# zdebruine/singlet

Measured on AMD Instinct MI355X. Metric: ALS iterations/sec (1M cells x 30k genes, 5% nnz, k=50), higher is better.
Workload: dtype f64

## Files before the change

### include/singlet_hip.h

```cpp
#ifndef SINGLET_HIP_H
#define SINGLET_HIP_H

#include <stddef.h>
#include <stdint.h>

#ifdef __cplusplus
extern "C" {
#endif

#define SGL_API __attribute__((visibility("default")))

#define SGL_OK 0
#define SGL_EINVAL (-1)
#define SGL_ENODEV (-2)
#define SGL_EHIP (-3)
#define SGL_ENOMEM (-4)
#define SGL_EINTR (-5)
#define SGL_ESTATE (-6)
#define SGL_ECOMM (-7)

SGL_API const char* sgl_last_error(void);
SGL_API int sgl_abi_version(void);
SGL_API int sgl_device_count(void);

// ... 282 lines not shown
SGL_API int sgl_comm_info(sgl_ctx* ctx, int32_t* nranks, int32_t* is_rccl, char* path_out, int path_len);
SGL_API int sgl_split_cells_by_nnz(const int32_t* p, int32_t ncol, int n, int64_t* lo);

SGL_API int sgl_op_rand(sgl_ctx* ctx, uint64_t state, const uint64_t* i, const uint64_t* j, int64_t n, uint64_t* out);
SGL_API int sgl_op_mask(sgl_ctx* ctx, uint64_t state, uint64_t inv_density, int64_t cell0, int32_t ncells, int32_t ngenes,
                uint8_t* out);
SGL_API int sgl_op_gram(sgl_ctx* ctx, const double* F, int32_t k, int64_t cols, double* G);
SGL_API int sgl_op_mask_gram(sgl_ctx* ctx, const double* F, const double* G, int32_t k, int32_t nrow, int64_t ncols, uint64_t seed,
                uint64_t inv_density, int mask_t, int64_t col_offset, int64_t row_offset, int use_lists, double* out);
SGL_API int sgl_op_rhs(sgl_ctx* ctx, int which, const double* F, int32_t k, double* B);
SGL_API int sgl_op_nnls(sgl_ctx* ctx, const double* G, const double* B, double* X, int32_t k, int64_t ncols,
                double L1, double L2, int32_t* sweeps_out);
SGL_API int sgl_op_transpose(sgl_ctx* ctx, int64_t max_batch_entries);
SGL_API int sgl_op_scale(sgl_ctx* ctx, double* F, int32_t k, int64_t cols, double* d);
SGL_API int sgl_op_cor(sgl_ctx* ctx, const double* x, const double* y, int64_t n, double* out);
SGL_API int sgl_op_graph_conv(sgl_ctx* ctx, const double* X, int32_t k, double* Y);
SGL_API int sgl_op_mse_test(sgl_ctx* ctx, uint64_t seed, uint64_t inv_density, double* out);
SGL_API int sgl_op_rhs_masked(sgl_ctx* ctx, int which, const double* F, int32_t k, uint64_t seed, uint64_t inv_density, double* B);
SGL_API int sgl_op_gene_mean(sgl_ctx* ctx, double* mean, int64_t* count);
SGL_API int sgl_op_gene_var(sgl_ctx* ctx, const double* mu, double* var);
SGL_API int sgl_op_gene_var_std(sgl_ctx* ctx, const double* mu, const double* sd, double vmax, double* out);
SGL_API int sgl_op_loess_direct(sgl_ctx* ctx, const double* x, const double* y, int64_t n, int64_t q, double* fitted);
SGL_API int sgl_op_marker_sums(sgl_ctx* ctx, const int32_t* labels, int32_t n_groups, int transform, int64_t* pos, int64_t* nz, double* sum);
SGL_API int sgl_op_marker_ranks(sgl_ctx* ctx, const int32_t* labels, int32_t n_groups, int64_t max_batch_entries, int64_t* rank2,
                                uint64_t* tie);
SGL_API int sgl_op_gsea_es(sgl_ctx* ctx, const double* w, int32_t m, int32_t k, const int64_t* set_ptr, const int32_t* set_genes,
                           int32_t n_sets, double* es_pos, double* es_neg, double* es_std);
SGL_API int sgl_op_gsea_null(sgl_ctx* ctx, const double* w, int32_t m, int32_t k, const int32_t* sizes, int32_t n_sizes,
                             int score_type, uint64_t seed, int32_t r0, int32_t r1, int32_t batch, double* null_out,
                             int32_t* sample);
// ... 28 lines not shown
```

### singlet_amd/_lib.py

```python
import ctypes as C
import os

_HERE = os.path.dirname(os.path.abspath(__file__))
LIB_PATH = os.environ.get("SGL_LIB_PATH", os.path.join(_HERE, "libsinglet_hip.so"))

SGL_PH_NAMES = ("gram", "rhs_h", "nnls_h", "rhs_w", "nnls_w", "scale", "comm", "mask", "mse")
SGL_PH_COUNT = len(SGL_PH_NAMES)

f64p = C.POINTER(C.c_double)
i32p = C.POINTER(C.c_int32)
i64p = C.POINTER(C.c_int64)
u64p = C.POINTER(C.c_uint64)
u8p = C.POINTER(C.c_uint8)

LOG_FN = C.CFUNCTYPE(None, C.c_void_p, C.c_int, C.c_double, C.c_double)
POLL_FN = C.CFUNCTYPE(C.c_int, C.c_void_p)
ALLREDUCE_FN = C.CFUNCTYPE(C.c_int, C.c_void_p, C.c_void_p, C.c_int64)


class Callbacks(C.Structure):
    _fields_ = [("user", C.c_void_p), ("log", LOG_FN), ("poll", POLL_FN)]


class SingletHipError(RuntimeError):
# ... 137 lines not shown
    "sgl_comm_available": (C.c_int, [C.c_char_p, C.c_int]),
    "sgl_comm_info": (C.c_int, [C.c_void_p, i32p, i32p, C.c_char_p, C.c_int]),
    "sgl_split_cells_by_nnz": (C.c_int, [i32p, C.c_int32, C.c_int, i64p]),
    "sgl_get_factors": (C.c_int, [C.c_void_p, f64p, f64p, f64p]),
    "sgl_set_factors": (C.c_int, [C.c_void_p, f64p, f64p, f64p]),
    "sgl_op_rand": (C.c_int, [C.c_void_p, C.c_uint64, u64p, u64p, C.c_int64, u64p]),
    "sgl_op_mask": (C.c_int, [C.c_void_p, C.c_uint64, C.c_uint64, C.c_int64, C.c_int32, C.c_int32, u8p]),
    "sgl_op_gram": (C.c_int, [C.c_void_p, f64p, C.c_int32, C.c_int64, f64p]),
    "sgl_op_rhs": (C.c_int, [C.c_void_p, C.c_int, f64p, C.c_int32, f64p]),
    "sgl_op_nnls": (C.c_int, [C.c_void_p, f64p, f64p, f64p, C.c_int32, C.c_int64, C.c_double, C.c_double, i32p]),
    "sgl_op_mask_gram": (C.c_int, [C.c_void_p, f64p, f64p, C.c_int32, C.c_int32, C.c_int64, C.c_uint64, C.c_uint64, C.c_int, C.c_int64,
                                   C.c_int64, C.c_int, f64p]),
    "sgl_op_transpose": (C.c_int, [C.c_void_p, C.c_int64]),
    "sgl_op_scale": (C.c_int, [C.c_void_p, f64p, C.c_int32, C.c_int64, f64p]),
    "sgl_op_cor": (C.c_int, [C.c_void_p, f64p, f64p, C.c_int64, f64p]),
    "sgl_op_graph_conv": (C.c_int, [C.c_void_p, f64p, C.c_int32, f64p]),
    "sgl_op_mse_test": (C.c_int, [C.c_void_p, C.c_uint64, C.c_uint64, f64p]),
    "sgl_op_rhs_masked": (C.c_int, [C.c_void_p, C.c_int, f64p, C.c_int32, C.c_uint64, C.c_uint64, f64p]),
    "sgl_op_gene_mean": (C.c_int, [C.c_void_p, f64p, i64p]),
    "sgl_op_gene_var": (C.c_int, [C.c_void_p, f64p, f64p]),
    "sgl_op_gene_var_std": (C.c_int, [C.c_void_p, f64p, f64p, C.c_double, f64p]),
    "sgl_op_loess_direct": (C.c_int, [C.c_void_p, f64p, f64p, C.c_int64, C.c_int64, f64p]),
    "sgl_op_nnls_percol": (C.c_int, [C.c_void_p, f64p, f64p, f64p, i64p, C.c_int32, C.c_int64, C.c_double, C.c_double, i32p]),
    "sgl_op_mse_test_cells": (C.c_int, [C.c_void_p, C.c_uint64, C.c_uint64, C.c_int, f64p]),
    "sgl_timing_enable": (C.c_int, [C.c_void_p, C.c_int]),
    "sgl_timing_get": (C.c_int, [C.c_void_p, f64p, i64p, C.c_int]),
    "sgl_sweeps_get": (C.c_int, [C.c_void_p, i64p, C.c_int]),
    "sgl_layout_get": (C.c_int, [C.c_void_p, i64p]),
    "sgl_layout_builds": (C.c_int, [C.c_void_p, i64p]),
    "sgl_mask_pairs": (C.c_int, [C.c_void_p, i64p]),
# ... 38 lines not shown
```

### singlet_amd/context.py

```python
import ctypes as C

import numpy as np

from . import _lib
from ._lib import check, f64p, i32p, i64p, ptr, u64p, u8p
from ._marshal import (MARKER_TRANSFORMS, ArdOutputs, NmfOutputs, colmajor, csc_ptrs, gsea_inputs, gsea_score_type, knn_call, label_list,
                       markers_call)
from .sparse import as_dgCMatrix

SYNTH_SEED = 0x5EED
LEVELS16 = np.log1p(1.0 + np.arange(16, dtype=np.float64))


def skew_weights16(sigma):
    z = np.array([-1.8627318674, -1.3180108973, -1.0099901692, -0.7764217611, -0.5791321623, -0.4022500653, -0.2372021093, -0.0784124127])
    z = np.concatenate([z, -z[::-1]])
    w = np.exp(float(sigma) * z)
    return w / w.mean()


def _f(a):
    return np.ascontiguousarray(a, dtype=np.float64)


# ... 506 lines not shown
        check(self._L.sgl_op_mask_gram(self._h, ptr(F, f64p), Gp, k, nrow, ncols, int(seed), int(inv_density), int(mask_t),
                                       int(col_offset), int(row_offset), 1 if use_lists else 0, ptr(out, f64p)))
        return out

    def op_transpose(self, max_batch_entries=0):
        check(self._L.sgl_op_transpose(self._h, int(max_batch_entries)))
        self.k = 0

    def op_scale(self, F):
        F = np.array(F, dtype=np.float64, order="C")
        cols, k = F.shape
        d = np.empty(k)
        check(self._L.sgl_op_scale(self._h, ptr(F, f64p), k, cols, ptr(d, f64p)))
        return F, d

    def op_cor(self, x, y):
        x, y = _f(x), _f(y)
        out = C.c_double()
        check(self._L.sgl_op_cor(self._h, ptr(x, f64p), ptr(y, f64p), x.size, C.byref(out)))
        return out.value

    def op_graph_conv(self, X, out=None):
        X = _f(X)
        n, k = X.shape
        _, nc, _ = self.dims()
        if n != nc:
            raise ValueError("X must have %d rows (the cells of the resident matrix)" % nc)
        Y = np.empty((n, k)) if out is None else out
        if Y.shape != (n, k) or Y.dtype != np.float64 or not Y.flags.c_contiguous:
            raise ValueError("out must be a C-contiguous float64 array of X's shape")
# ... 202 lines not shown
```

### singlet_amd/csrc/kernels_dense.hip

```cpp
#include "sgl_internal.h"

typedef double d4 __attribute__((ext_vector_type(4)));

template <int NT>
__global__ __launch_bounds__(256) void gram_mfma_kernel(const double* __restrict__ F, int k, int64_t cols,
                                                        int64_t cols_per_block, double* __restrict__ part) {
    constexpr int NTILES = NT * (NT + 1) / 2;
    const int lane = threadIdx.x & 63, wave = threadIdx.x >> 6;
    const int r16 = lane & 15, kk = lane >> 4;
    const int64_t c_begin = (int64_t)blockIdx.x * cols_per_block;
    int64_t c_end = c_begin + cols_per_block;
    if (c_end > cols) c_end = cols;

    d4 acc[NTILES];
#pragma unroll
    for (int t = 0; t < NTILES; ++t) acc[t] = d4{0, 0, 0, 0};

    for (int64_t c = c_begin + 4 * wave; c < c_end; c += 16) {
        const int64_t cc = c + kk;
        double f[NT];
#pragma unroll
        for (int b = 0; b < NT; ++b) {
            const int row = b * 16 + r16;
            f[b] = (cc < c_end && row < k) ? F[cc * k + row] : 0.0;
        }
        int t = 0;
#pragma unroll
        for (int bi = 0; bi < NT; ++bi)
#pragma unroll
            for (int bj = 0; bj <= bi; ++bj) {
                acc[t] = __builtin_amdgcn_mfma_f64_16x16x4f64(f[bi], f[bj], acc[t], 0, 0, 0);
                ++t;
            }
    }

    __shared__ double sm[4][64 * 4];
    double* out = part + (size_t)blockIdx.x * k * k;
    int t = 0;
#pragma unroll
    for (int bi = 0; bi < NT; ++bi)
#pragma unroll
        for (int bj = 0; bj <= bi; ++bj) {
            __syncthreads();
#pragma unroll
            for (int r = 0; r < 4; ++r) sm[wave][lane * 4 + r] = acc[t][r];
            __syncthreads();
            if (wave == 0) {
#pragma unroll
// ... 170 lines not shown
        partial_sum_small_kernel<<<dim3(1), dim3(1024), 0, c->stream>>>(c->ws, nblocks, n, nseg, add_all, out);
        HIPCHK(hipGetLastError());
        return SGL_OK;
    }
    if (add_all != 0.0) { sgl_set_error("partial sum: add_all only in the short form"); return SGL_EINVAL; }
    double* tmp = c->ws + (size_t)nblocks * n;
    partial_sum_stage1_kernel<<<dim3((n + 255) / 256, nseg), dim3(256), 0, c->stream>>>(c->ws, nblocks, n, tmp);
    HIPCHK(hipGetLastError());
    partial_sum_stage2_kernel<<<dim3((n + 255) / 256), dim3(256), 0, c->stream>>>(tmp, nseg, n, diag_k, diag_add, out);
    HIPCHK(hipGetLastError());
    return SGL_OK;
}

int k_gram_big_partials(hipStream_t s, const double* F, int k, int64_t cols, int64_t cols_per_block, int nblocks, double* part);

int k_gram(sgl_ctx* c, const double* F, int k, int64_t cols, double* G, double diag_add) {
    if (k <= 0 || k > SGL_MAX_K) { sgl_set_error("k_gram: k=%d out of range", k); return SGL_EINVAL; }
    int nblocks = (int)((cols + 255) / 256);
    if (nblocks > 1024) nblocks = 1024;
    const bool big_mfma = k > 128 && k <= 256 && !getenv("SGL_GRAM_BIG_VALU");
    if (k > 128 && nblocks > (big_mfma ? 512 : 128)) nblocks = big_mfma ? 512 : 128;
    if (nblocks < 1) nblocks = 1;
    int64_t cpb = (cols + nblocks - 1) / nblocks;
    cpb = (cpb + 15) / 16 * 16;
    nblocks = (int)((cols + cpb - 1) / cpb);
    if (nblocks < 1) nblocks = 1;
    SGLCHK(sgl_ws_reserve(c, sizeof(double) * sgl_partial_ws(nblocks, k * k)));
    hipStream_t s = c->stream;
    const int NT = (k + 15) / 16;
    if (NT == 1) gram_mfma_kernel<1><<<dim3(nblocks), dim3(256), 0, s>>>(F, k, cols, cpb, c->ws);
    else if (NT == 2) gram_mfma_kernel<2><<<dim3(nblocks), dim3(256), 0, s>>>(F, k, cols, cpb, c->ws);
    else if (NT == 3) gram_mfma_kernel<3><<<dim3(nblocks), dim3(256), 0, s>>>(F, k, cols, cpb, c->ws);
    else if (NT == 4) gram_mfma_kernel<4><<<dim3(nblocks), dim3(256), 0, s>>>(F, k, cols, cpb, c->ws);
    else if (NT == 5) gram_mfma_split_kernel<5><<<dim3(nblocks), dim3(256), 0, s>>>(F, k, cols, cpb, c->ws);
    else if (NT == 6) gram_mfma_split_kernel<6><<<dim3(nblocks), dim3(256), 0, s>>>(F, k, cols, cpb, c->ws);
    else if (NT == 7) gram_mfma_split_kernel<7><<<dim3(nblocks), dim3(256), 0, s>>>(F, k, cols, cpb, c->ws);
    else if (NT == 8) gram_mfma_split_kernel<8><<<dim3(nblocks), dim3(256), 0, s>>>(F, k, cols, cpb, c->ws);
    else if (big_mfma) SGLCHK(k_gram_big_partials(s, F, k, cols, cpb, nblocks, c->ws));
    else {
        const size_t lds = sizeof(double) * 16 * (size_t)k;
        if (lds > 48 * 1024) HIPCHK(hipFuncSetAttribute(reinterpret_cast<const void*>(&gram_valu_kernel), hipFuncAttributeMaxDynamicSharedMemorySize, 144 * 1024));
        for (int pair0 = 0; pair0 < k * k; pair0 += 256 * GV_MAXP)
            gram_valu_kernel<<<dim3(nblocks), dim3(256), lds, s>>>(F, k, cols, cpb, c->ws, pair0);
    }
    HIPCHK(hipGetLastError());
    return sgl_partial_sum(c, nblocks, k * k, k, diag_add, G);
}

// ... 72 lines not shown

int k_scale_apply(hipStream_t s, double* F, int k, int64_t cols, double* d, int add_eps) {
    if (add_eps) {
        add_eps_kernel<<<dim3((k + 63) / 64), dim3(64), 0, s>>>(d, k);
        HIPCHK(hipGetLastError());
    }
    const int64_t n = (int64_t)k * cols;
    if (n <= 0) return SGL_OK;
    int64_t blocks = (n + 255) / 256;
    if (blocks > 4096) blocks = 4096;
    scale_kernel<<<dim3((unsigned)blocks), dim3(256), 0, s>>>(F, k, n, d);
    HIPCHK(hipGetLastError());
    return SGL_OK;
}

__global__ __launch_bounds__(256) void cor_partial_kernel(const double* __restrict__ x, const double* __restrict__ y,
                                                          int64_t n, double* __restrict__ part) {
    double s[5] = {0, 0, 0, 0, 0};
    for (int64_t t = (int64_t)blockIdx.x * blockDim.x + threadIdx.x; t < n; t += (int64_t)gridDim.x * blockDim.x) {
        const double a = x[t], b = y[t];
        s[0] += a;
        s[1] += b;
        s[2] = fma(a, b, s[2]);
        s[3] = fma(a, a, s[3]);
        s[4] = fma(b, b, s[4]);
    }
    __shared__ double sm[5][256];
    for (int q = 0; q < 5; ++q) sm[q][threadIdx.x] = s[q];
    __syncthreads();
    for (int w = 128; w > 0; w >>= 1) {
// ... 122 lines not shown
```

### singlet_amd/csrc/sgl_internal.h

```cpp
#pragma once
#include <hip/hip_runtime.h>
#include <stdint.h>
#include <stdio.h>
#include <stdarg.h>
#include <atomic>
#include <functional>
#include <vector>
#include <algorithm>

#include "../../include/singlet_hip.h"

#define SGL_WAVE 64
#define SGL_MAX_K 1024
#define SGL_LANE_NNLS_MAX_K 128

void sgl_set_error(const char* fmt, ...);

hipError_t sgl_pool_malloc_raw(void** p, size_t bytes);
template <typename T_>
inline hipError_t sgl_pool_malloc(T_** p, size_t bytes) { return sgl_pool_malloc_raw(reinterpret_cast<void**>(p), bytes); }
hipError_t sgl_pool_free(void* p);
hipError_t sgl_pool_mem_info(size_t* free_b, size_t* total_b);
void sgl_pool_release(void);
size_t sgl_pool_cached_bytes(void);
// ... 150 lines not shown
    hipStream_t stream = nullptr;

    DevCSC A, At;
    DevTiled TA, TAt;
    bool use_tiled = false;
    int64_t cell_offset = 0, ncells_total = 0;
    int64_t* col_nnz_A = nullptr;
    int64_t* col_nnz_At = nullptr;
    int64_t* col_nnz_At_global = nullptr;
    bool gene_nnz_global = false;

    int k = 0;
    double *W = nullptr, *Wprev = nullptr, *H = nullptr, *d = nullptr;
    double* B = nullptr;
    double* red = nullptr;
    double* G = nullptr;
    double* Gpad = nullptr;
    NnlsScratch nnls_scr;
    bool solve_empty = false;
    double* Adense = nullptr;
    bool dense_gemm = false;
    void* rocblas = nullptr;
    double* link_h = nullptr;
    double* link_w = nullptr;
    int link_h_rows = 0, link_w_rows = 0;
    DevGroupLink glink_h, glink_w;
    DevGraph graph;
    bool dense_input = false;
    DevMaskList ML[2];
    int64_t ml_builds[2] = {0, 0};
// ... 118 lines not shown
                 const double* skew_dev = nullptr);
int k_synth_winit(hipStream_t s, uint64_t S, int k, int32_t ngenes, double* W);
int k_exclusive_scan(sgl_ctx* c, const int64_t* in, int64_t* out, int64_t n);
int k_scan_total(hipStream_t s, const int64_t* in, int64_t* out, int64_t n);
int k_col_counts(hipStream_t s, const int64_t* p, int64_t ncol, int64_t* counts);
int k_validate_csc(hipStream_t s, const int32_t* idx, const int64_t* p, int64_t ncol, int32_t nrow, int* flag_dev);
int k_all_finite(hipStream_t s, const double* x, int64_t n, int* flag_dev);
int k_widen_p(hipStream_t s, const int32_t* p32, int64_t n1, int64_t* p64);
int k_build_segments(hipStream_t s, const DevCSC& M);

int k_gram(sgl_ctx* c, const double* F, int k, int64_t cols, double* G, double diag_add);
int k_gram_add_diag(hipStream_t s, double* G, int k, double v);
int k_rowsum(sgl_ctx* c, const double* F, int k, int64_t cols, double* d_out, int add_eps = 0);
bool k_rowsum_can_add_eps(int k, int64_t cols);
int k_scale_apply(hipStream_t s, double* F, int k, int64_t cols, double* d, int add_eps);
int k_cor(sgl_ctx* c, const double* x, const double* y, int64_t n, double* out_dev);
int k_pad_gram(hipStream_t s, const double* G, int k, int KP, int GS, double* Gpad);
int k_gram_rescale(hipStream_t s, double* G, int k, const double* d, double diag_add);
int k_i64_to_f64(hipStream_t s, const int64_t* in, double* out, int64_t n);
int k_f64_to_i64(hipStream_t s, const double* in, int64_t* out, int64_t n);
int k_transpose_dense(hipStream_t s, const double* in, int rows, int cols, double* out);

int k_acc(hipStream_t s, const DevCSC& M, const double* F, int k, double* B,
          uint64_t mask_seed, uint64_t inv_density, int mask_mode, int64_t mask_col_offset, int64_t mask_row_offset);

void sgl_tiled_free(DevTiled& S);
int sgl_tiled_build(sgl_ctx* c, const DevCSC& M, int k, DevTiled& S);
int k_acc_tiled(hipStream_t s, const DevTiled& S, const double* F, int ldf, double* B, int ldb, int kf, const double* xvals = nullptr);
int k_acc_tiled_all(hipStream_t s, const DevTiled& S, const double* F, double* B, int k, const double* xvals = nullptr);
int sgl_tiled_mask_values(sgl_ctx* c, const DevCSC& M, DevTiled& S, uint64_t seed, uint64_t inv_density, int mask_t,
// ... 167 lines not shown
```

### singlet_amd/csrc/singlet_hip.hip

```cpp
#include "sgl_internal.h"
#include "ingest_host.h"

#include <math.h>
#include <string.h>
#include <algorithm>
#include <string>
#include <chrono>
#include <mutex>
#include <vector>
#include <stdlib.h>

static thread_local char g_err[1024] = "";

void sgl_set_error(const char* fmt, ...) {
    va_list ap;
    va_start(ap, fmt);
    vsnprintf(g_err, sizeof(g_err), fmt, ap);
    va_end(ap);
}

extern "C" const char* sgl_last_error(void) { return g_err; }
extern "C" int sgl_abi_version(void) { return 2; }

struct CallTimes {
// ... 143 lines not shown
    dev_free(c->Wd);
    dev_free(c->Sbuf);
    dev_free(c->Stri);
    nnls_scratch_free(c->nnls_scr);
    links_clear(c);
    free_graph(c);
    dev_free(c->A.seg);
    dev_free(c->At.seg);
    if (!keep_streams) {
        sgl_tiled_free(c->TA);
        sgl_tiled_free(c->TAt);
        sgl_mask_lists_free_all(c);
    }
    c->use_tiled = false;
    c->k = 0;
}

static void free_matrix(sgl_ctx* c) {
    sgl_dense_release(c);
    free_csc(c->A);
    free_csc(c->At);
    dev_free(c->col_nnz_A);
    dev_free(c->col_nnz_At);
    dev_free(c->col_nnz_At_global);
    c->gene_nnz_global = false;
    c->dense_input = false;
}

static int drop_matrix(sgl_ctx* c, int rc) {
    (void)hipStreamSynchronize(c->stream);
// ... 755 lines not shown
    if (rc == SGL_OK) rc = sgl_download_csc(c, 0, x_out, nullptr, nullptr);
    sgl_destroy(c);
    return rc;
}

static int64_t team_gene_block(const sgl_ctx* c) {
    const int64_t m = c->A.nrow;
    const int n = sgl_team_size(c);
    return n > 1 ? (m + n - 1) / n : m;
}

static int fit_init_impl(sgl_ctx* c, int32_t k, const double* w_init, uint64_t synth_seed) {
    const int64_t m = c->A.nrow, n = c->A.ncol;
    const int64_t mpad = team_gene_block(c) * std::max(1, sgl_team_size(c));
    sgl_trace_setup(nullptr);
    SGLCHK(dev_alloc(&c->W, (size_t)k * mpad + 2));
    SGLCHK(dev_alloc(&c->Wprev, (size_t)k * m));
    SGLCHK(dev_alloc(&c->H, (size_t)k * n + 2));
    SGLCHK(dev_alloc(&c->d, (size_t)k));
    SGLCHK(dev_alloc(&c->B, (size_t)k * n + 2));
    SGLCHK(dev_alloc(&c->red, (size_t)k * mpad + (size_t)k * k + (size_t)k));
    SGLCHK(dev_alloc(&c->G, (size_t)k * k));
    SGLCHK(dev_alloc(&c->Gpad, (size_t)SGL_LANE_NNLS_MAX_K * (SGL_LANE_NNLS_MAX_K + 16) + 64));
    {
        const int64_t cap = std::max<int64_t>(c->A.ncol, c->A.nrow);
        if (k <= SGL_LANE_NNLS_MAX_K) SGLCHK(nnls_scratch_alloc(c->nnls_scr, cap, k));
        if (k <= 256 && c->A.ncol >= 65536) SGLCHK(nnls_pack_alloc(c->nnls_scr, c->A.ncol));
    }
    sgl_trace_setup("fit: factor buffers allocated");
    HIPCHK(hipMemsetAsync(c->W, 0, sizeof(double) * ((size_t)k * mpad + 2), c->stream));
// ... 93 lines not shown
    if (k > SGL_LANE_NNLS_MAX_K && k <= 256 && h_side && ncols == c->A.ncol && ncols >= 65536 && c->nnls_scr.prev_it != nullptr &&
        !getenv("SGL_NNLS_NO_QUARTER"))
        return k_nnls_quarter_packed(c->stream, G, B, X, col_nnz, k, ncols, L1, L2, counter, &c->nnls_scr);
    return k_nnls_percol(c->stream, G, 0, B, X, col_nnz, k, ncols, L1, L2, counter);
}

extern "C" int sgl_step_begin(sgl_ctx* c) {
    FIT_GUARD(c);
    Phase ph(c, SGL_PH_SCALE);
    HIPCHK(hipMemcpyAsync(c->Wprev, c->W, sizeof(double) * (size_t)c->k * c->A.nrow, hipMemcpyDeviceToDevice, c->stream));
    return SGL_OK;
}

int sgl_step_h_rhs(sgl_ctx* c, bool convolve) {
    const int k = c->k;
    { Phase ph(c, SGL_PH_GRAM); SGLCHK(k_gram(c, c->W, k, c->A.nrow, c->G, 1e-15)); }
    { Phase ph(c, SGL_PH_RHS_H);
      if (c->dense_gemm) SGLCHK(k_dense_rhs(c, 0, c->W, k, c->B));
      else if (c->use_tiled) SGLCHK(k_acc_tiled_all(c->stream, c->TA, c->W, c->B, k));
      else SGLCHK(k_acc(c->stream, c->A, c->W, k, c->B, 0, 1, 0, 0, 0));
      if (c->link_h) SGLCHK(k_link_mul(c->stream, c->B, c->link_h, k, c->link_h_rows, c->A.ncol));
      else if (c->glink_h.table) SGLCHK(k_link_mul_grouped(c->stream, c->B, c->glink_h.table, c->glink_h.group, k, c->glink_h.rows, c->glink_h.groups, c->A.ncol));
      if (c->graph.n && convolve) SGLCHK(k_graph_conv(c->stream, c->graph, c->B, c->graph.buf, k)); }
    return SGL_OK;
}

int sgl_step_h_solve(sgl_ctx* c, double L1, double L2, bool convolve) {
    const int k = c->k;
    if (c->graph.n && convolve) { Phase ph(c, SGL_PH_RHS_H); SGLCHK(k_graph_conv(c->stream, c->graph, c->B, c->graph.buf, k)); }
    { Phase ph(c, SGL_PH_NNLS_H);
      if (c->graph.n) SGLCHK(sgl_nnls_shared(c, c->G, c->graph.buf, c->H, nullptr, c->A.ncol, L1, L2, c->sweep_counters + 0, true));
      else SGLCHK(sgl_nnls_shared(c, c->G, c->B, c->H, c->solve_empty ? nullptr : c->col_nnz_A, c->A.ncol, L1, L2, c->sweep_counters + 0, true)); }
    return SGL_OK;
}

extern "C" int sgl_step_h(sgl_ctx* c, double L1, double L2) {
    FIT_GUARD(c);
    SGLCHK(sgl_step_h_rhs(c, true));
    return sgl_step_h_solve(c, L1, L2, false);
}

extern "C" int sgl_step_scale_h(sgl_ctx* c) {
    FIT_GUARD(c);
    if (c->team && sgl_team_size(c) > 1) { sgl_set_error("step API on a native team: use sgl_nmf_iterate / sgl_multi_iterate"); return SGL_ESTATE; }
    const int eps_in_sum = (!c->allreduce && k_rowsum_can_add_eps(c->k, c->A.ncol)) ? 1 : 0;
    { Phase ph(c, SGL_PH_SCALE); SGLCHK(k_rowsum(c, c->H, c->k, c->A.ncol, c->d, eps_in_sum)); }
    SGLCHK(do_allreduce(c, c->d, c->k));
    { Phase ph(c, SGL_PH_SCALE); SGLCHK(k_scale_apply(c->stream, c->H, c->k, c->A.ncol, c->d, eps_in_sum ? 0 : 1)); }
    return SGL_OK;
}

extern "C" int sgl_step_w(sgl_ctx* c, double L1, double L2) {
    FIT_GUARD(c);
    if (c->team && sgl_team_size(c) > 1) { sgl_set_error("step API on a native team: use sgl_nmf_iterate / sgl_multi_iterate"); return SGL_ESTATE; }
    const int k = c->k;
    const int64_t m = c->A.nrow;
    double* Bw = c->red;
    double* Gh = c->red + (size_t)k * m;
    const int64_t* gene_nnz = nullptr;
    SGLCHK(gene_counts(c, &gene_nnz));
    { Phase ph(c, SGL_PH_RHS_W);
      const double* F = c->H;
      if (c->graph.n) { SGLCHK(k_graph_conv(c->stream, c->graph, c->H, c->B, k)); F = c->B; }
      if (c->dense_gemm) SGLCHK(k_dense_rhs(c, 1, F, k, Bw));
      else if (c->use_tiled && c->TAt.roff) SGLCHK(k_acc_tiled_all(c->stream, c->TAt, F, Bw, k));
      else SGLCHK(k_acc(c->stream, c->At, F, k, Bw, 0, 1, 0, 0, 0)); }
    { Phase ph(c, SGL_PH_GRAM); SGLCHK(k_gram(c, c->H, k, c->A.ncol, Gh, 0.0)); }
    SGLCHK(do_allreduce(c, c->red, (int64_t)k * m + (int64_t)k * k));
    { Phase ph(c, SGL_PH_GRAM);
      HIPCHK(hipMemcpyAsync(c->G, Gh, sizeof(double) * k * k, hipMemcpyDeviceToDevice, c->stream));
      SGLCHK(k_gram_add_diag(c->stream, c->G, k, 1e-15)); }
    { Phase ph(c, SGL_PH_NNLS_W);
      if (c->link_w) SGLCHK(k_link_mul(c->stream, Bw, c->link_w, k, c->link_w_rows, m));
      else if (c->glink_w.table) SGLCHK(k_link_mul_grouped(c->stream, Bw, c->glink_w.table, c->glink_w.group, k, c->glink_w.rows, c->glink_w.groups, m));
      SGLCHK(sgl_nnls_shared(c, c->G, Bw, c->W, (c->solve_empty || c->graph.n) ? nullptr : gene_nnz, m, L1, L2, c->sweep_counters + 1)); }
    return SGL_OK;
}

int sgl_scale_w_enqueue(sgl_ctx* c) {
    const int k = c->k;
    const int64_t m = c->A.nrow;
    Phase ph(c, SGL_PH_SCALE);
// ... 27 lines not shown
    c->wave_sweeps_acc[0] += h[2];
    c->wave_sweeps_acc[1] += h[3];
    return SGL_OK;
}

static bool interrupted(const sgl_callbacks* cb) {
    if (!(cb && cb->poll && cb->poll(cb->user))) return false;
    sgl_set_error("interrupted");
    return true;
}

int sgl_iterate_shard(sgl_ctx* c, double L1_w, double L1_h, double L2_w, double L2_h, const ArdArgs* mask, const sgl_callbacks* cb,
                      double* tol) {
    SGLCHK(sgl_step_begin(c));
    SGLCHK(mask ? sgl_step_h_masked(c, L1_h, L2_h, mask->seed, mask->inv_density) : sgl_step_h(c, L1_h, L2_h));
    SGLCHK(sgl_step_scale_h(c));
    if (interrupted(cb)) return SGL_EINTR;
    SGLCHK(mask ? sgl_step_w_masked(c, L1_w, L2_w, mask->seed, mask->inv_density) : sgl_step_w(c, L1_w, L2_w));
    return sgl_step_scale_w(c, tol);
}

int sgl_als_loop(double tol, int32_t maxit, const std::function<int(double*)>& iterate, const ArdArgs* ard,
                 const std::function<int(double*)>& mse_test, sgl_ctx* const* ctxs, int nctx, double* tol_trace, int32_t* n_iter,
                 const sgl_callbacks* cb) {
    double tol_ = 1.0;
    int it = 0, nt = 0;
    auto push_trace = [&](int iter_now) -> int {
        double err = 0.0;
        SGLCHK(mse_test(&err));
        ard->test_mse[nt] = err;
        ard->iter[nt] = iter_now;
// ... 43 lines not shown
    HIPCHK(hipStreamSynchronize(c->stream));
    return SGL_OK;
}

extern "C" int sgl_get_factors(sgl_ctx* c, double* w, double* d, double* h) {
    FIT_GUARD(c);
    HIPCHK(hipStreamSynchronize(c->stream));
    if (w) HIPCHK(hipMemcpy(w, c->W, sizeof(double) * (size_t)c->k * c->A.nrow, hipMemcpyDeviceToHost));
    if (d) HIPCHK(hipMemcpy(d, c->d, sizeof(double) * (size_t)c->k, hipMemcpyDeviceToHost));
    if (h) HIPCHK(hipMemcpy(h, c->H, sizeof(double) * (size_t)c->k * c->A.ncol, hipMemcpyDeviceToHost));
    return SGL_OK;
}

extern "C" int sgl_set_factors(sgl_ctx* c, const double* w, const double* d, const double* h) {
    FIT_GUARD(c);
    HIPCHK(hipStreamSynchronize(c->stream));
    if (w) HIPCHK(hipMemcpy(c->W, w, sizeof(double) * (size_t)c->k * c->A.nrow, hipMemcpyHostToDevice));
    if (d) HIPCHK(hipMemcpy(c->d, d, sizeof(double) * (size_t)c->k, hipMemcpyHostToDevice));
    if (h) HIPCHK(hipMemcpy(c->H, h, sizeof(double) * (size_t)c->k * c->A.ncol, hipMemcpyHostToDevice));
    return SGL_OK;
}

int sgl_mask_workspace(sgl_ctx* c) {
    const int k = c->k;
    if (!c->Gcols) {
        const int64_t widest = std::max<int64_t>(c->A.ncol, c->At.ncol);
        size_t free_b = 0, total_b = 0;
        HIPCHK(sgl_pool_mem_info(&free_b, &total_b));
        const char* e = getenv("SGL_GCOLS_MB");
        const int64_t mb = (e && atoll(e) > 0) ? atoll(e) : std::min<int64_t>(16384, std::max<int64_t>(256, (int64_t)(free_b >> 23)));
// ... 12 lines not shown
    const DevCSC& M = orientation ? c->At : c->A;
    DevTiled& S = orientation ? c->TAt : c->TA;
    const int64_t col_off = mask_t ? 0 : c->cell_offset;
    const int64_t row_off = mask_t ? c->cell_offset : 0;
    if (c->use_tiled && S.roff && !getenv("SGL_MASKED_RHS_PLAIN")) {
        SGLCHK(sgl_tiled_mask_values(c, M, S, seed, inv_density, mask_t, col_off, row_off));
        return k_acc_tiled_all(c->stream, S, F, Bbuf, c->k, S.xm);
    }
    return k_acc(c->stream, M, F, c->k, Bbuf, seed, inv_density, mask_t ? 2 : 1, col_off, row_off);
}

int sgl_predict_mask_dev(sgl_ctx* c, const DevCSC& M, const int64_t* col_nnz, const double* F, double* X,
                            double* Bbuf, uint64_t seed, uint64_t inv_density, double L1, double L2, int mask_t,
                            int rhs_phase, int nnls_phase, unsigned long long* counter) {
    const int k = c->k;
    SGLCHK(sgl_mask_workspace(c));
    const int64_t col_off = mask_t ? 0 : c->cell_offset;
    const int64_t row_off = mask_t ? c->cell_offset : 0;
    { Phase ph(c, SGL_PH_GRAM); SGLCHK(k_gram(c, F, k, M.nrow, c->G, 1e-15)); }
    { Phase ph(c, rhs_phase);
      SGLCHK(sgl_masked_rhs(c, mask_t, F, Bbuf, seed, inv_density)); }
    const int64_t chunk = c->gcols_chunk;
    DevMaskList* L = nullptr;
    if (k <= 128 && !getenv("SGL_MASK_NO_LIST")) {
        Phase ph(c, SGL_PH_MASK);
        DevMaskList& Lm = c->ML[mask_t ? 1 : 0];
        SGLCHK(sgl_mask_list_select(c, mask_t ? 1 : 0, M.ncol, M.nrow, seed, inv_density, mask_t, col_off, row_off));
        if (Lm.mask_t == mask_t) L = &Lm;
    }
    for (int64_t c0 = 0; c0 < M.ncol; c0 += chunk) {
// ... 1055 lines not shown

extern "C" int sgl_op_scale(sgl_ctx* c, double* F, int32_t k, int64_t cols, double* d) {
    CTX_GUARD(c);
    if (!F || !d || k <= 0 || cols < 0) { sgl_set_error("sgl_op_scale: bad arguments"); return SGL_EINVAL; }
    DevBuf<double> dF, dd;
    SGLCHK(dF.alloc((size_t)k * cols));
    SGLCHK(dd.alloc((size_t)k));
    HIPCHK(hipMemcpyAsync(dF.p, F, sizeof(double) * (size_t)k * cols, hipMemcpyHostToDevice, c->stream));
    int rc = k_rowsum(c, dF.p, k, cols, dd.p);
    if (rc == SGL_OK) rc = k_scale_apply(c->stream, dF.p, k, cols, dd.p, 1);
    if (rc == SGL_OK && (hipMemcpyAsync(F, dF.p, sizeof(double) * (size_t)k * cols, hipMemcpyDeviceToHost, c->stream) != hipSuccess ||
                         hipMemcpyAsync(d, dd.p, sizeof(double) * (size_t)k, hipMemcpyDeviceToHost, c->stream) != hipSuccess)) rc = SGL_EHIP;
    return op_finish(c, rc, "sgl_op_scale");
}

extern "C" int sgl_op_cor(sgl_ctx* c, const double* x, const double* y, int64_t n, double* out) {
    CTX_GUARD(c);
    if (!x || !y || !out || n <= 0) { sgl_set_error("sgl_op_cor: bad arguments"); return SGL_EINVAL; }
    DevBuf<double> dx, dy;
    SGLCHK(dx.alloc((size_t)n));
    SGLCHK(dy.alloc((size_t)n));
    HIPCHK(hipMemcpyAsync(dx.p, x, sizeof(double) * (size_t)n, hipMemcpyHostToDevice, c->stream));
    HIPCHK(hipMemcpyAsync(dy.p, y, sizeof(double) * (size_t)n, hipMemcpyHostToDevice, c->stream));
    int rc = k_cor(c, dx.p, dy.p, n, c->scalars + 2);
    if (rc == SGL_OK && hipMemcpyAsync(out, c->scalars + 2, sizeof(double), hipMemcpyDeviceToHost, c->stream) != hipSuccess) rc = SGL_EHIP;
    return op_finish(c, rc, "sgl_op_cor");
}

extern "C" int sgl_op_graph_conv(sgl_ctx* c, const double* X, int32_t k, double* Y) {
    FIT_GUARD(c);
// ... 77 lines not shown
```

Before: 43.09.

## Fuse H scaling with H Gram computation and prefetch columns in gram kernel

Adds a SCALE variant of the MFMA gram kernel that divides each H column by d, writes it back and accumulates the Gram in the same pass. The W step then reuses the cached H Gram through a validity flag instead of recomputing it. This removes one full read/write pass over H (scale) plus a separate Gram read. The gram kernel also gains a register prefetch ring of depth SGL_GRAM_AHEAD, which hides load latency at the cost of extra registers. The cache flag must be invalidated on every path that mutates H, so missing an invalidation would reuse a stale Gram.

```diff
diff --git a/include/singlet_hip.h b/include/singlet_hip.h
--- a/include/singlet_hip.h
+++ b/include/singlet_hip.h
@@ -320,6 +320,7 @@
 SGL_API int sgl_op_transpose(sgl_ctx* ctx, int64_t max_batch_entries);
 SGL_API int sgl_op_scale(sgl_ctx* ctx, double* F, int32_t k, int64_t cols, double* d);
 SGL_API int sgl_op_cor(sgl_ctx* ctx, const double* x, const double* y, int64_t n, double* out);
+SGL_API int sgl_op_scale_gram(sgl_ctx* ctx, double* F, int32_t k, int64_t cols, double* d, double* G);
 SGL_API int sgl_op_graph_conv(sgl_ctx* ctx, const double* X, int32_t k, double* Y);
 SGL_API int sgl_op_mse_test(sgl_ctx* ctx, uint64_t seed, uint64_t inv_density, double* out);
 SGL_API int sgl_op_rhs_masked(sgl_ctx* ctx, int which, const double* F, int32_t k, uint64_t seed, uint64_t inv_density, double* B);
diff --git a/singlet_amd/_lib.py b/singlet_amd/_lib.py
--- a/singlet_amd/_lib.py
+++ b/singlet_amd/_lib.py
@@ -175,6 +175,7 @@
     "sgl_op_transpose": (C.c_int, [C.c_void_p, C.c_int64]),
     "sgl_op_scale": (C.c_int, [C.c_void_p, f64p, C.c_int32, C.c_int64, f64p]),
     "sgl_op_cor": (C.c_int, [C.c_void_p, f64p, f64p, C.c_int64, f64p]),
+    "sgl_op_scale_gram": (C.c_int, [C.c_void_p, f64p, C.c_int32, C.c_int64, f64p, f64p]),
     "sgl_op_graph_conv": (C.c_int, [C.c_void_p, f64p, C.c_int32, f64p]),
     "sgl_op_mse_test": (C.c_int, [C.c_void_p, C.c_uint64, C.c_uint64, f64p]),
     "sgl_op_rhs_masked": (C.c_int, [C.c_void_p, C.c_int, f64p, C.c_int32, C.c_uint64, C.c_uint64, f64p]),
diff --git a/singlet_amd/context.py b/singlet_amd/context.py
--- a/singlet_amd/context.py
+++ b/singlet_amd/context.py
@@ -544,6 +544,14 @@
         check(self._L.sgl_op_scale(self._h, ptr(F, f64p), k, cols, ptr(d, f64p)))
         return F, d
 
+    def op_scale_gram(self, F):
+        F = np.array(F, dtype=np.float64, order="C")
+        cols, k = F.shape
+        d = np.empty(k)
+        G = np.empty((k, k))
+        check(self._L.sgl_op_scale_gram(self._h, ptr(F, f64p), k, cols, ptr(d, f64p), ptr(G, f64p)))
+        return F, d, G
+
     def op_cor(self, x, y):
         x, y = _f(x), _f(y)
         out = C.c_double()
diff --git a/singlet_amd/csrc/kernels_dense.hip b/singlet_amd/csrc/kernels_dense.hip
--- a/singlet_amd/csrc/kernels_dense.hip
+++ b/singlet_amd/csrc/kernels_dense.hip
@@ -2,10 +2,18 @@
 
 typedef double d4 __attribute__((ext_vector_type(4)));
 
-template <int NT>
-__global__ __launch_bounds__(256) void gram_mfma_kernel(const double* __restrict__ F, int k, int64_t cols,
-                                                        int64_t cols_per_block, double* __restrict__ part) {
+#ifndef SGL_GRAM_AHEAD
+#define SGL_GRAM_AHEAD 2
+#endif
+template <bool SCALE> struct gram_operand { typedef const double* __restrict__ ptr; };
+template <> struct gram_operand<true> { typedef double* ptr; };
+
+template <int NT, bool SCALE>
+__global__ __launch_bounds__(256) void gram_mfma_kernel(typename gram_operand<SCALE>::ptr F, int k, int64_t cols,
+                                                        int64_t cols_per_block, const double* __restrict__ d,
+                                                        double* __restrict__ part) {
     constexpr int NTILES = NT * (NT + 1) / 2;
+    constexpr int AH = SGL_GRAM_AHEAD;
     const int lane = threadIdx.x & 63, wave = threadIdx.x >> 6;
     const int r16 = lane & 15, kk = lane >> 4;
     const int64_t c_begin = (int64_t)blockIdx.x * cols_per_block;
@@ -16,22 +24,56 @@
 #pragma unroll
     for (int t = 0; t < NTILES; ++t) acc[t] = d4{0, 0, 0, 0};
 
-    for (int64_t c = c_begin + 4 * wave; c < c_end; c += 16) {
-        const int64_t cc = c + kk;
-        double f[NT];
-#pragma unroll
-        for (int b = 0; b < NT; ++b) {
-            const int row = b * 16 + r16;
-            f[b] = (cc < c_end && row < k) ? F[cc * k + row] : 0.0;
-        }
-        int t = 0;
-#pragma unroll
-        for (int bi = 0; bi < NT; ++bi)
-#pragma unroll
-            for (int bj = 0; bj <= bi; ++bj) {
-                acc[t] = __builtin_amdgcn_mfma_f64_16x16x4f64(f[bi], f[bj], acc[t], 0, 0, 0);
-                ++t;
+    double dv[NT];
+#pragma unroll
+    for (int b = 0; b < NT; ++b) {
+        const int row = b * 16 + r16;
+        dv[b] = (SCALE && row < k) ? d[row] : 1.0;
+    }
+
+    double q[AH + 1][NT];
+    int64_t roff[NT];
+#pragma unroll
+    for (int b = 0; b < NT; ++b) roff[b] = (b * 16 + r16 < k) ? b * 16 + r16 : k - 1;
+    if (c_begin < c_end) {
+#pragma unroll
+        for (int a = 0; a < AH; ++a) {
+            const int64_t cc = c_begin + 4 * wave + 16 * a + kk;
+            const int64_t cl = (cc < c_end) ? cc : c_end - 1;
+#pragma unroll
+            for (int b = 0; b < NT; ++b) q[a][b] = F[cl * k + roff[b]];
+        }
+    }
+    for (int64_t c = c_begin + 4 * wave; c < c_end;) {
+#pragma unroll
+        for (int j = 0; j <= AH; ++j) {
+            if (c >= c_end) break;
+            const int64_t cc = c + kk, cn = cc + 16 * AH;
+            const int64_t cl = (cn < c_end) ? cn : c_end - 1;
+            double* nxt = q[(j + AH) % (AH + 1)];
+#pragma unroll
+            for (int b = 0; b < NT; ++b) nxt[b] = F[cl * k + roff[b]];
+            double f[NT];
+#pragma unroll
+            for (int b = 0; b < NT; ++b) {
+                const bool mine = cc < c_end && b * 16 + r16 < k;
+                f[b] = q[j][b];
+                if constexpr (SCALE) {
+                    f[b] = f[b] / dv[b];
+                    if (mine) F[cc * k + b * 16 + r16] = f[b];
+                }
+                f[b] = mine ? f[b] : 0.0;
             }
+            int t = 0;
+#pragma unroll
+            for (int bi = 0; bi < NT; ++bi)
+#pragma unroll
+                for (int bj = 0; bj <= bi; ++bj) {
+                    acc[t] = __builtin_amdgcn_mfma_f64_16x16x4f64(f[bi], f[bj], acc[t], 0, 0, 0);
+                    ++t;
+                }
+            c += 16;
+        }
     }
 
     __shared__ double sm[4][64 * 4];
@@ -232,24 +274,32 @@
 
 int k_gram_big_partials(hipStream_t s, const double* F, int k, int64_t cols, int64_t cols_per_block, int nblocks, double* part);
 
-int k_gram(sgl_ctx* c, const double* F, int k, int64_t cols, double* G, double diag_add) {
-    if (k <= 0 || k > SGL_MAX_K) { sgl_set_error("k_gram: k=%d out of range", k); return SGL_EINVAL; }
+static void gram_partition(int k, int64_t cols, bool big_mfma, int* nblocks_out, int64_t* cpb_out) {
     int nblocks = (int)((cols + 255) / 256);
     if (nblocks > 1024) nblocks = 1024;
-    const bool big_mfma = k > 128 && k <= 256 && !getenv("SGL_GRAM_BIG_VALU");
     if (k > 128 && nblocks > (big_mfma ? 512 : 128)) nblocks = big_mfma ? 512 : 128;
     if (nblocks < 1) nblocks = 1;
     int64_t cpb = (cols + nblocks - 1) / nblocks;
     cpb = (cpb + 15) / 16 * 16;
     nblocks = (int)((cols + cpb - 1) / cpb);
     if (nblocks < 1) nblocks = 1;
+    *nblocks_out = nblocks;
+    *cpb_out = cpb;
+}
+
+int k_gram(sgl_ctx* c, const double* F, int k, int64_t cols, double* G, double diag_add) {
+    if (k <= 0 || k > SGL_MAX_K) { sgl_set_error("k_gram: k=%d out of range", k); return SGL_EINVAL; }
+    const bool big_mfma = k > 128 && k <= 256 && !getenv("SGL_GRAM_BIG_VALU");
+    int nblocks;
+    int64_t cpb;
+    gram_partition(k, cols, big_mfma, &nblocks, &cpb);
     SGLCHK(sgl_ws_reserve(c, sizeof(double) * sgl_partial_ws(nblocks, k * k)));
     hipStream_t s = c->stream;
     const int NT = (k + 15) / 16;
-    if (NT == 1) gram_mfma_kernel<1><<<dim3(nblocks), dim3(256), 0, s>>>(F, k, cols, cpb, c->ws);
-    else if (NT == 2) gram_mfma_kernel<2><<<dim3(nblocks), dim3(256), 0, s>>>(F, k, cols, cpb, c->ws);
-    else if (NT == 3) gram_mfma_kernel<3><<<dim3(nblocks), dim3(256), 0, s>>>(F, k, cols, cpb, c->ws);
-    else if (NT == 4) gram_mfma_kernel<4><<<dim3(nblocks), dim3(256), 0, s>>>(F, k, cols, cpb, c->ws);
+    if (NT == 1) gram_mfma_kernel<1, false><<<dim3(nblocks), dim3(256), 0, s>>>(F, k, cols, cpb, nullptr, c->ws);
+    else if (NT == 2) gram_mfma_kernel<2, false><<<dim3(nblocks), dim3(256), 0, s>>>(F, k, cols, cpb, nullptr, c->ws);
+    else if (NT == 3) gram_mfma_kernel<3, false><<<dim3(nblocks), dim3(256), 0, s>>>(F, k, cols, cpb, nullptr, c->ws);
+    else if (NT == 4) gram_mfma_kernel<4, false><<<dim3(nblocks), dim3(256), 0, s>>>(F, k, cols, cpb, nullptr, c->ws);
     else if (NT == 5) gram_mfma_split_kernel<5><<<dim3(nblocks), dim3(256), 0, s>>>(F, k, cols, cpb, c->ws);
     else if (NT == 6) gram_mfma_split_kernel<6><<<dim3(nblocks), dim3(256), 0, s>>>(F, k, cols, cpb, c->ws);
     else if (NT == 7) gram_mfma_split_kernel<7><<<dim3(nblocks), dim3(256), 0, s>>>(F, k, cols, cpb, c->ws);
@@ -352,6 +402,32 @@
     return SGL_OK;
 }
 
+bool k_scale_gram_fused(int k) { return k <= 64 && !getenv("SGL_NO_SCALE_GRAM_FUSE"); }
+
+int k_scale_gram(sgl_ctx* c, double* F, int k, int64_t cols, double* d, int add_eps, double* G, double diag_add) {
+    if (k <= 0 || k > SGL_MAX_K) { sgl_set_error("k_scale_gram: k=%d out of range", k); return SGL_EINVAL; }
+    if (!k_scale_gram_fused(k)) {
+        SGLCHK(k_scale_apply(c->stream, F, k, cols, d, add_eps));
+        return k_gram(c, F, k, cols, G, diag_add);
+    }
+    hipStream_t s = c->stream;
+    if (add_eps) {
+        add_eps_kernel<<<dim3((k + 63) / 64), dim3(64), 0, s>>>(d, k);
+        HIPCHK(hipGetLastError());
+    }
+    int nblocks;
+    int64_t cpb;
+    gram_partition(k, cols, false, &nblocks, &cpb);
+    SGLCHK(sgl_ws_reserve(c, sizeof(double) * sgl_partial_ws(nblocks, k * k)));
+    const int NT = (k + 15) / 16;
+    if (NT == 1) gram_mfma_kernel<1, true><<<dim3(nblocks), dim3(256), 0, s>>>(F, k, cols, cpb, d, c->ws);
+    else if (NT == 2) gram_mfma_kernel<2, true><<<dim3(nblocks), dim3(256), 0, s>>>(F, k, cols, cpb, d, c->ws);
+    else if (NT == 3) gram_mfma_kernel<3, true><<<dim3(nblocks), dim3(256), 0, s>>>(F, k, cols, cpb, d, c->ws);
+    else gram_mfma_kernel<4, true><<<dim3(nblocks), dim3(256), 0, s>>>(F, k, cols, cpb, d, c->ws);
+    HIPCHK(hipGetLastError());
+    return sgl_partial_sum(c, nblocks, k * k, k, diag_add, G);
+}
+
 __global__ __launch_bounds__(256) void cor_partial_kernel(const double* __restrict__ x, const double* __restrict__ y,
                                                           int64_t n, double* __restrict__ part) {
     double s[5] = {0, 0, 0, 0, 0};
diff --git a/singlet_amd/csrc/sgl_internal.h b/singlet_amd/csrc/sgl_internal.h
--- a/singlet_amd/csrc/sgl_internal.h
+++ b/singlet_amd/csrc/sgl_internal.h
@@ -188,6 +188,7 @@
     double *W = nullptr, *Wprev = nullptr, *H = nullptr, *d = nullptr;
     double* B = nullptr;
     double* red = nullptr;
+    bool gh_valid = false;
     double* G = nullptr;
     double* Gpad = nullptr;
     NnlsScratch nnls_scr;
@@ -336,6 +337,8 @@
 int k_rowsum(sgl_ctx* c, const double* F, int k, int64_t cols, double* d_out, int add_eps = 0);
 bool k_rowsum_can_add_eps(int k, int64_t cols);
 int k_scale_apply(hipStream_t s, double* F, int k, int64_t cols, double* d, int add_eps);
+int k_scale_gram(sgl_ctx* c, double* F, int k, int64_t cols, double* d, int add_eps, double* G, double diag_add);
+bool k_scale_gram_fused(int k);
 int k_cor(sgl_ctx* c, const double* x, const double* y, int64_t n, double* out_dev);
 int k_pad_gram(hipStream_t s, const double* G, int k, int KP, int GS, double* Gpad);
 int k_gram_rescale(hipStream_t s, double* G, int k, const double* d, double diag_add);
diff --git a/singlet_amd/csrc/singlet_hip.hip b/singlet_amd/csrc/singlet_hip.hip
--- a/singlet_amd/csrc/singlet_hip.hip
+++ b/singlet_amd/csrc/singlet_hip.hip
@@ -181,6 +181,7 @@
     }
     c->use_tiled = false;
     c->k = 0;
+    c->gh_valid = false;
 }
 
 static void free_matrix(sgl_ctx* c) {
@@ -966,6 +967,7 @@
     const int64_t m = c->A.nrow, n = c->A.ncol;
     const int64_t mpad = team_gene_block(c) * std::max(1, sgl_team_size(c));
     sgl_trace_setup(nullptr);
+    c->gh_valid = false;
     SGLCHK(dev_alloc(&c->W, (size_t)k * mpad + 2));
     SGLCHK(dev_alloc(&c->Wprev, (size_t)k * m));
     SGLCHK(dev_alloc(&c->H, (size_t)k * n + 2));
@@ -1089,6 +1091,7 @@
 
 int sgl_step_h_rhs(sgl_ctx* c, bool convolve) {
     const int k = c->k;
+    c->gh_valid = false;
     { Phase ph(c, SGL_PH_GRAM); SGLCHK(k_gram(c, c->W, k, c->A.nrow, c->G, 1e-15)); }
     { Phase ph(c, SGL_PH_RHS_H);
       if (c->dense_gemm) SGLCHK(k_dense_rhs(c, 0, c->W, k, c->B));
@@ -1102,6 +1105,7 @@
 
 int sgl_step_h_solve(sgl_ctx* c, double L1, double L2, bool convolve) {
     const int k = c->k;
+    c->gh_valid = false;
     if (c->graph.n && convolve) { Phase ph(c, SGL_PH_RHS_H); SGLCHK(k_graph_conv(c->stream, c->graph, c->B, c->graph.buf, k)); }
     { Phase ph(c, SGL_PH_NNLS_H);
       if (c->graph.n) SGLCHK(sgl_nnls_shared(c, c->G, c->graph.buf, c->H, nullptr, c->A.ncol, L1, L2, c->sweep_counters + 0, true));
@@ -1115,14 +1119,23 @@
     return sgl_step_h_solve(c, L1, L2, false);
 }
 
-extern "C" int sgl_step_scale_h(sgl_ctx* c) {
-    FIT_GUARD(c);
+static int scale_h(sgl_ctx* c, bool with_gram) {
     if (c->team && sgl_team_size(c) > 1) { sgl_set_error("step API on a native team: use sgl_nmf_iterate / sgl_multi_iterate"); return SGL_ESTATE; }
+    c->gh_valid = false;
     const int eps_in_sum = (!c->allreduce && k_rowsum_can_add_eps(c->k, c->A.ncol)) ? 1 : 0;
     { Phase ph(c, SGL_PH_SCALE); SGLCHK(k_rowsum(c, c->H, c->k, c->A.ncol, c->d, eps_in_sum)); }
     SGLCHK(do_allreduce(c, c->d, c->k));
-    { Phase ph(c, SGL_PH_SCALE); SGLCHK(k_scale_apply(c->stream, c->H, c->k, c->A.ncol, c->d, eps_in_sum ? 0 : 1)); }
-    return SGL_OK;
+    Phase ph(c, SGL_PH_SCALE);
+    if (with_gram && !c->graph.n && c->A.ncol > 0 && k_scale_gram_fused(c->k)) {
+        SGLCHK(k_scale_gram(c, c->H, c->k, c->A.ncol, c->d, eps_in_sum ? 0 : 1, c->red + (size_t)c->k * c->A.nrow, 0.0));
+        c->gh_valid = true;
+    } else SGLCHK(k_scale_apply(c->stream, c->H, c->k, c->A.ncol, c->d, eps_in_sum ? 0 : 1));
+    return SGL_OK;
+}
+
+extern "C" int sgl_step_scale_h(sgl_ctx* c) {
+    FIT_GUARD(c);
+    return scale_h(c, true);
 }
 
 extern "C" int sgl_step_w(sgl_ctx* c, double L1, double L2) {
@@ -1140,7 +1153,9 @@
       if (c->dense_gemm) SGLCHK(k_dense_rhs(c, 1, F, k, Bw));
       else if (c->use_tiled && c->TAt.roff) SGLCHK(k_acc_tiled_all(c->stream, c->TAt, F, Bw, k));
       else SGLCHK(k_acc(c->stream, c->At, F, k, Bw, 0, 1, 0, 0, 0)); }
-    { Phase ph(c, SGL_PH_GRAM); SGLCHK(k_gram(c, c->H, k, c->A.ncol, Gh, 0.0)); }
+    const bool have_gh = c->gh_valid && !c->graph.n;
+    c->gh_valid = false;
+    if (!have_gh) { Phase ph(c, SGL_PH_GRAM); SGLCHK(k_gram(c, c->H, k, c->A.ncol, Gh, 0.0)); }
     SGLCHK(do_allreduce(c, c->red, (int64_t)k * m + (int64_t)k * k));
     { Phase ph(c, SGL_PH_GRAM);
       HIPCHK(hipMemcpyAsync(c->G, Gh, sizeof(double) * k * k, hipMemcpyDeviceToDevice, c->stream));
@@ -1198,7 +1213,8 @@
                       double* tol) {
     SGLCHK(sgl_step_begin(c));
     SGLCHK(mask ? sgl_step_h_masked(c, L1_h, L2_h, mask->seed, mask->inv_density) : sgl_step_h(c, L1_h, L2_h));
-    SGLCHK(sgl_step_scale_h(c));
+    FIT_GUARD(c);
+    SGLCHK(scale_h(c, mask == nullptr));
     if (interrupted(cb)) return SGL_EINTR;
     SGLCHK(mask ? sgl_step_w_masked(c, L1_w, L2_w, mask->seed, mask->inv_density) : sgl_step_w(c, L1_w, L2_w));
     return sgl_step_scale_w(c, tol);
@@ -1272,6 +1288,7 @@
 
 extern "C" int sgl_set_factors(sgl_ctx* c, const double* w, const double* d, const double* h) {
     FIT_GUARD(c);
+    c->gh_valid = false;
     HIPCHK(hipStreamSynchronize(c->stream));
     if (w) HIPCHK(hipMemcpy(c->W, w, sizeof(double) * (size_t)c->k * c->A.nrow, hipMemcpyHostToDevice));
     if (d) HIPCHK(hipMemcpy(c->d, d, sizeof(double) * (size_t)c->k, hipMemcpyHostToDevice));
@@ -1314,6 +1331,7 @@
                             double* Bbuf, uint64_t seed, uint64_t inv_density, double L1, double L2, int mask_t,
                             int rhs_phase, int nnls_phase, unsigned long long* counter) {
     const int k = c->k;
+    c->gh_valid = false;
     SGLCHK(sgl_mask_workspace(c));
     const int64_t col_off = mask_t ? 0 : c->cell_offset;
     const int64_t row_off = mask_t ? c->cell_offset : 0;
@@ -2399,6 +2417,22 @@
     return op_finish(c, rc, "sgl_op_scale");
 }
 
+extern "C" int sgl_op_scale_gram(sgl_ctx* c, double* F, int32_t k, int64_t cols, double* d, double* G) {
+    CTX_GUARD(c);
+    if (!F || !d || !G || k <= 0 || cols <= 0) { sgl_set_error("sgl_op_scale_gram: bad arguments"); return SGL_EINVAL; }
+    DevBuf<double> dF, dd, dG;
+    SGLCHK(dF.alloc((size_t)k * cols));
+    SGLCHK(dd.alloc((size_t)k));
+    SGLCHK(dG.alloc((size_t)k * k));
+    HIPCHK(hipMemcpyAsync(dF.p, F, sizeof(double) * (size_t)k * cols, hipMemcpyHostToDevice, c->stream));
+    int rc = k_rowsum(c, dF.p, k, cols, dd.p);
+    if (rc == SGL_OK) rc = k_scale_gram(c, dF.p, k, cols, dd.p, 1, dG.p, 1e-15);
+    if (rc == SGL_OK && (hipMemcpyAsync(F, dF.p, sizeof(double) * (size_t)k * cols, hipMemcpyDeviceToHost, c->stream) != hipSuccess ||
+                         hipMemcpyAsync(d, dd.p, sizeof(double) * (size_t)k, hipMemcpyDeviceToHost, c->stream) != hipSuccess ||
+                         hipMemcpyAsync(G, dG.p, sizeof(double) * (size_t)k * k, hipMemcpyDeviceToHost, c->stream) != hipSuccess)) rc = SGL_EHIP;
+    return op_finish(c, rc, "sgl_op_scale_gram");
+}
+
 extern "C" int sgl_op_cor(sgl_ctx* c, const double* x, const double* y, int64_t n, double* out) {
     CTX_GUARD(c);
     if (!x || !y || !out || n <= 0) { sgl_set_error("sgl_op_cor: bad arguments"); return SGL_EINVAL; }
```

Result: no change. 43.44, median of 6 (+0.8%).
